# masapasa/qcpinn-convection-diffusion-qiskit

Measured on AMD Instinct MI355X. Metric: collocation-points/sec (PDE+BC+IC loss step), 4-qubit cascade, higher is better.
Workload: dtype f32

## Files before the change

### qcpinn-convection-diffusion-qiskit_amd/csrc/qc_mlp.hip

```cpp
#include "qc_internal.h"
#include "qc_philox.h"

namespace {

__device__ __forceinline__ float qc_tanh(float x) {
  const float e = __expf(2.f * x);
  return 1.f - 2.f * __builtin_amdgcn_rcpf(e + 1.f);
}

typedef float mf2 __attribute__((ext_vector_type(2)));
__device__ __forceinline__ mf2 m_dup(const float a) { return (mf2){a, a}; }
__device__ __forceinline__ mf2 m_fma(const mf2 a, const mf2 b, const mf2 c) { return __builtin_elementwise_fma(a, b, c); }

__device__ __forceinline__ float analytic_u(float t, float x, float y) {
  const float dx = x - 0.5f, dy = y - 0.5f;
  return expf(-100.f * (dx * dx + dy * dy)) * expf(-t);
}
__device__ __forceinline__ float analytic_r(float t, float x, float y, float D, float vx, float vy) {
  const float u = analytic_u(t, x, y);
  const float dx = x - 0.5f, dy = y - 0.5f;
  const float ut = -u, ux = -200.f * dx * u, uy = -200.f * dy * u;
  const float uxx = (40000.f * dx * dx - 400.f) * u;
  const float uyy = (40000.f * dy * dy - 400.f) * u;
  return ut + vx * ux + vy * uy - D * (uxx + uyy);
}

__device__ __forceinline__ float analytic_u_diffusion(float t, float x, float y, float D) {
  const float pi = 3.14159265358979323846f;
  return sinf(pi * x) * sinf(pi * y) * expf(-2.f * pi * pi * D * t);
}

__device__ __forceinline__ float residual_target(const QcPde& pde, float t, float x, float y) {
  return pde.problem != QC_PB_CONVECTION_DIFFUSION ? 0.f : analytic_r(t, x, y, pde.D, pde.vx, pde.vy);
}
__device__ __forceinline__ float value_target(const QcPde& pde, bool seg_a, float t, float x, float y) {
  return pde.problem == QC_PB_PURE_DIFFUSION ? (seg_a ? analytic_u_diffusion(t, x, y, pde.D) : 0.f) : analytic_u(t, x, y);
}

constexpr float QC_PI_F = 3.14159265358979323846f;

template <int NCH>
__device__ __forceinline__ void angle_map_fwd(const float (&v)[NCH], float (&a)[NCH]) {
  const float tau = qc_tanh(v[0]);
  const float ps = QC_PI_F * (1.f - tau * tau);
  a[0] = QC_PI_F * tau;
  if constexpr (NCH == 6) {
    a[1] = ps * v[1];
    a[2] = ps * v[2];
    a[3] = ps * v[3];
    a[4] = ps * (v[4] - 2.f * tau * v[2] * v[2]);
    a[5] = ps * (v[5] - 2.f * tau * v[3] * v[3]);
  }
}

template <int NCH>
__device__ __forceinline__ void angle_map_bwd(const float (&ab)[NCH], const float (&a)[NCH], float (&vb)[NCH]) {
  const float tau = a[0] * (1.f / QC_PI_F);
  const float ps = QC_PI_F * (1.f - tau * tau);
  vb[0] = ps * ab[0];
  if constexpr (NCH == 6) {
    const float tt = 2.f * tau;
    vb[1] = ps * ab[1];
    vb[2] = ps * ab[2] - 2.f * tt * a[2] * ab[4];
    vb[3] = ps * ab[3] - 2.f * tt * a[3] * ab[5];
    vb[4] = ps * ab[4];
    vb[5] = ps * ab[5];
    vb[0] -= tt * (a[1] * ab[1] + a[2] * ab[2] + a[3] * ab[3]) +
             (tt * a[4] + 2.f * a[2] * a[2] * (1.f / QC_PI_F)) * ab[4] +
             (tt * a[5] + 2.f * a[3] * a[3] * (1.f / QC_PI_F)) * ab[5];
  }
}

constexpr int QC_MS = 4;

template <int N, int NCH, int MAP = 0, bool RF = false>
__device__ __forceinline__ void k_pre_fwd_body(const int64_t bid, const float* __restrict__ X, const float* __restrict__ prm,
                                                 QcLayout L, float* __restrict__ ajets, int64_t B,
                                                 const QcDraw* __restrict__ draw = nullptr, float* __restrict__ Xout = nullptr) {
  __shared__ float s_part[QC_MS][NCH * N][64];
  const int lane = threadIdx.x & 63;
  const int wave = __builtin_amdgcn_readfirstlane(threadIdx.x >> 6);
  const int64_t p = (int64_t)bid * 64 + lane;
  const int64_t pc = p < B ? p : B - 1;
  float t, x, y;
  if (draw != nullptr && draw->enabled) {
    if (NCH == 6) qc_draw_point(0, draw->off_res + pc, 0, draw->seed, draw->step, t, x, y);
    else if (pc < draw->n_ic) qc_draw_point(1, draw->off_ic + pc, 0, draw->seed, draw->step, t, x, y);
    else qc_draw_point<RF>(2, draw->off_bc + (pc - draw->n_ic), draw->face_pts, draw->seed, draw->step, t, x, y);
    if (wave == 0 && p < B) {
      Xout[p * 3 + 0] = t;
      Xout[p * 3 + 1] = x;
      Xout[p * 3 + 2] = y;
    }
  } else {
    t = X[pc * 3 + 0];
    x = X[pc * 3 + 1];
    y = X[pc * 3 + 2];
  }
  constexpr int NP2 = NCH == 6 ? 3 : 1;
  mf2 acc2[NP2][N];
#pragma unroll
  for (int cp = 0; cp < NP2; ++cp)
#pragma unroll
    for (int i = 0; i < N; ++i) acc2[cp][i] = (mf2){0.f, 0.f};
  const float* W1 = prm + L.oW1;
  const float* b1 = prm + L.ob1;
  const float* W2 = prm + L.oW2;
  const int hq = (L.H + QC_MS - 1) / QC_MS;
  const int m0 = wave * hq, m1 = (m0 + hq) < L.H ? (m0 + hq) : L.H;
  for (int m = m0; m < m1; ++m) {
    const float w0 = W1[3 * m], w1 = W1[3 * m + 1], w2 = W1[3 * m + 2];
    const float h = fmaf(w0, t, fmaf(w1, x, fmaf(w2, y, b1[m])));
    const float z = qc_tanh(h);
    if constexpr (NCH == 6) {
      const float d1 = 1.f - z * z, d2 = -2.f * z * d1;
      const mf2 zc2[3] = {(mf2){z, d1 * w0}, (mf2){d1 * w1, d1 * w2}, (mf2){d2 * w1 * w1, d2 * w2 * w2}};
#pragma unroll
      for (int i = 0; i < N; ++i) {
        const mf2 wi = m_dup(W2[i * L.H + m]);
#pragma unroll
        for (int cp = 0; cp < 3; ++cp) acc2[cp][i] = m_fma(wi, zc2[cp], acc2[cp][i]);
      }
    } else {
#pragma unroll
      for (int i = 0; i < N; ++i) acc2[0][i].x = fmaf(W2[i * L.H + m], z, acc2[0][i].x);
    }
  }
#pragma unroll
  for (int c = 0; c < NCH; ++c)
#pragma unroll
    for (int i = 0; i < N; ++i) s_part[wave][c * N + i][lane] = (c & 1) ? acc2[c >> 1][i].y : acc2[c >> 1][i].x;
  __syncthreads();
  if (p < B) {
    if constexpr (MAP == 0) {
      for (int f = wave; f < NCH * N; f += QC_MS) {
        float v = (s_part[0][f][lane] + s_part[1][f][lane]) + (s_part[2][f][lane] + s_part[3][f][lane]);
        if (f < N) v += prm[L.ob2 + f];
        ajets[(int64_t)f * B + p] = v;
      }
    } else {
      for (int i = wave; i < N; i += QC_MS) {
        float v[NCH], a[NCH];
#pragma unroll
        for (int c = 0; c < NCH; ++c) {
          const int f = c * N + i;
          v[c] = (s_part[0][f][lane] + s_part[1][f][lane]) + (s_part[2][f][lane] + s_part[3][f][lane]);
        }
        v[0] += prm[L.ob2 + i];
        angle_map_fwd<NCH>(v, a);
#pragma unroll
        for (int c = 0; c < NCH; ++c) ajets[(int64_t)(c * N + i) * B + p] = a[c];
      }
    }
  }
}

template <int N, int NCH, int MAP>
__global__ void __launch_bounds__(256) k_pre_fwd(const float* __restrict__ X, const float* __restrict__ prm,
                                                 QcLayout L, float* __restrict__ ajets, int64_t B) {
  k_pre_fwd_body<N, NCH, MAP>(blockIdx.x, X, prm, L, ajets, B);
}

template <int N, int NCH, int MAP = 0>
__device__ __forceinline__ void k_pre_bwd_body(const int64_t bid, const float* __restrict__ X, const float* __restrict__ prm, QcLayout L,
                          const float* __restrict__ abar, float* __restrict__ part, int64_t part_stride,
                          int64_t row0, int64_t B, int HB, int PS, const float* __restrict__ aj = nullptr) {
  constexpr int NP2 = NCH == 6 ? 3 : 1;
  __shared__ float sX[3][64];
  __shared__ mf2 sA2[NP2 * N][64];
  extern __shared__ float s_acc[];
  const int64_t base = (int64_t)bid * 64;
  const int cnt = (int)((B - base) < 64 ? (B - base) : 64);
  for (int i = threadIdx.x; i < 64 * 3; i += blockDim.x) {
    const int pp = i / 3, k = i % 3;
    sX[k][pp] = pp < cnt ? X[(base + pp) * 3 + k] : 0.f;
  }
  if constexpr (MAP == 0) {
    for (int i = threadIdx.x; i < NCH * N * 64; i += blockDim.x) {
      const int f = i >> 6, pp = i & 63;
      const int c = f / N, w = f % N;
      const float v = pp < cnt ? abar[(int64_t)f * B + base + pp] : 0.f;
      if (c & 1) sA2[(c >> 1) * N + w][pp].y = v;
      else sA2[(c >> 1) * N + w][pp].x = v;
    }
  } else {
    for (int i = threadIdx.x; i < N * 64; i += blockDim.x) {
      const int w = i >> 6, pp = i & 63;
      float ab[NCH], a[NCH], vb[NCH];
#pragma unroll
      for (int c = 0; c < NCH; ++c) {
        const int64_t o = (int64_t)(c * N + w) * B + base + pp;
        ab[c] = pp < cnt ? abar[o] : 0.f;
        a[c] = pp < cnt ? aj[o] : 0.f;
      }
      angle_map_bwd<NCH>(ab, a, vb);
#pragma unroll
      for (int c = 0; c < NCH; ++c) {
        if (c & 1) sA2[(c >> 1) * N + w][pp].y = vb[c];
        else sA2[(c >> 1) * N + w][pp].x = vb[c];
      }
    }
  }
  __syncthreads();

  const int grp = threadIdx.x / HB, m = threadIdx.x % HB;
  const int per = (64 + PS - 1) / PS;
  const int p0 = grp * per, p1 = (p0 + per) < cnt ? (p0 + per) : cnt;
  float gW1[3] = {0.f, 0.f, 0.f}, gb1 = 0.f;
  mf2 gW2p[N];
#pragma unroll
  for (int i = 0; i < N; ++i) gW2p[i] = (mf2){0.f, 0.f};
  if (grp < PS && m < L.H) {
    const float w0 = prm[L.oW1 + 3 * m], w1 = prm[L.oW1 + 3 * m + 1], w2 = prm[L.oW1 + 3 * m + 2];
    const float bb = prm[L.ob1 + m];
    float w2c[N];
#pragma unroll
    for (int i = 0; i < N; ++i) w2c[i] = prm[L.oW2 + i * L.H + m];
    for (int pp = p0; pp < p1; ++pp) {
      const float t = sX[0][pp], x = sX[1][pp], y = sX[2][pp];
      const float h = fmaf(w0, t, fmaf(w1, x, fmaf(w2, y, bb)));
      const float z = qc_tanh(h);
      const float d1 = 1.f - z * z;
      if constexpr (NCH == 6) {
        mf2 a2[3][N], zb2[3];
#pragma unroll
        for (int cp = 0; cp < 3; ++cp) {
          zb2[cp] = (mf2){0.f, 0.f};
#pragma unroll
          for (int i = 0; i < N; ++i) {
            a2[cp][i] = sA2[cp * N + i][pp];
            zb2[cp] = m_fma(m_dup(w2c[i]), a2[cp][i], zb2[cp]);
          }
        }
        const float d2 = -2.f * z * d1;
        const float d3 = -2.f * (d1 * d1 + z * d2);
        const mf2 zc2[3] = {(mf2){z, d1 * w0}, (mf2){d1 * w1, d1 * w2}, (mf2){d2 * w1 * w1, d2 * w2 * w2}};
#pragma unroll
        for (int i = 0; i < N; ++i)
#pragma unroll
          for (int cp = 0; cp < 3; ++cp) gW2p[i] = m_fma(a2[cp][i], zc2[cp], gW2p[i]);
        const float zb[6] = {zb2[0].x, zb2[0].y, zb2[1].x, zb2[1].y, zb2[2].x, zb2[2].y};
        const float hb = zb[0] * d1 + (zb[1] * w0 + zb[2] * w1 + zb[3] * w2) * d2 +
                         (zb[4] * w1 * w1 + zb[5] * w2 * w2) * d3;
        gW1[0] += hb * t + zb[1] * d1;
        gW1[1] += hb * x + zb[2] * d1 + 2.f * zb[4] * d2 * w1;
        gW1[2] += hb * y + zb[3] * d1 + 2.f * zb[5] * d2 * w2;
        gb1 += hb;
      } else {
        float zb0 = 0.f;
#pragma unroll
        for (int i = 0; i < N; ++i) {
          const float a = sA2[i][pp].x;
          zb0 = fmaf(w2c[i], a, zb0);
          gW2p[i].x = fmaf(a, z, gW2p[i].x);
        }
        const float hb = zb0 * d1;
        gW1[0] += hb * t;
        gW1[1] += hb * x;
        gW1[2] += hb * y;
        gb1 += hb;
      }
    }
  }
  if (grp < PS) {
    float* mine = s_acc + (size_t)grp * (4 + N) * HB;
    mine[0 * HB + m] = gW1[0];
    mine[1 * HB + m] = gW1[1];
    mine[2 * HB + m] = gW1[2];
    mine[3 * HB + m] = gb1;
#pragma unroll
    for (int i = 0; i < N; ++i) mine[(4 + i) * HB + m] = gW2p[i].x + gW2p[i].y;
  }
  __syncthreads();
  float* row = part + (row0 + bid) * part_stride;
  if (grp == 0 && m < L.H) {
    float tot[4 + N];
#pragma unroll
    for (int k = 0; k < 4 + N; ++k) {
      float sum = 0.f;
      for (int g2 = 0; g2 < PS; ++g2) sum += s_acc[((size_t)g2 * (4 + N) + k) * HB + m];
      tot[k] = sum;
    }
    row[L.oW1 + 3 * m] = tot[0];
    row[L.oW1 + 3 * m + 1] = tot[1];
    row[L.oW1 + 3 * m + 2] = tot[2];
    row[L.ob1 + m] = tot[3];
#pragma unroll
    for (int i = 0; i < N; ++i) row[L.oW2 + i * L.H + m] = tot[4 + i];
  }
  if (threadIdx.x < N) {
    float sum = 0.f;
// ... 229 lines not shown
    __syncthreads();
    if (live) {
      for (int f = wave; f < NCH * N; f += QC_MS)
        qbar[(int64_t)f * B + p] = (s_buf[0][f][lane] + s_buf[1][f][lane]) + (s_buf[2][f][lane] + s_buf[3][f][lane]);
    }
  }
}

template <int N, int NCH, int MODE>
__global__ void __launch_bounds__(256) k_post(const float* __restrict__ X, const float* __restrict__ prm, QcLayout L,
                                              QcPde pde, const float* __restrict__ qjets,
                                              float* __restrict__ out_u, float* __restrict__ out_res,
                                              const float* __restrict__ in_ubar, const float* __restrict__ in_rbar,
                                              float* __restrict__ qbar, float* __restrict__ part,
                                              int64_t part_stride, int64_t row0, int64_t B) {
  k_post_body<N, NCH, MODE>(blockIdx.x, X, prm, L, pde, qjets, out_u, out_res, in_ubar, in_rbar, qbar, part, part_stride, row0, B);
}

template <int N, int NCH>
__device__ __forceinline__ void k_post_wg_body(const int64_t bid, const float* __restrict__ prm, QcLayout L, QcPde pde, const float* __restrict__ qjets,
                          const float* __restrict__ ubar, const float* __restrict__ rbar,
                          float* __restrict__ part, int64_t part_stride, int64_t row0, int64_t B, int HB, int PS,
                          int gen = 0) {
  __shared__ float sQ[NCH * N][64];
  __shared__ float sU[NCH == 6 ? 6 : 2][64];
  extern __shared__ float s_acc[];
  const int64_t base = (int64_t)bid * 64;
  const int cnt = (int)((B - base) < 64 ? (B - base) : 64);
  for (int i = threadIdx.x; i < NCH * N * 64; i += blockDim.x) {
    const int f = i >> 6, pp = i & 63;
    sQ[f][pp] = pp < cnt ? qjets[(int64_t)f * B + base + pp] : 0.f;
  }
  if (NCH == 6 && gen) {
    for (int i = threadIdx.x; i < 6 * 64; i += blockDim.x) {
      const int k = i >> 6, pp = i & 63;
      sU[k][pp] = pp < cnt ? ubar[(int64_t)k * B + base + pp] : 0.f;
    }
  } else {
    for (int i = threadIdx.x; i < 128; i += blockDim.x) {
      const int k = i >> 6, pp = i & 63;
      const float* src = k == 0 ? ubar : rbar;
      sU[k][pp] = (pp < cnt && src != nullptr) ? src[base + pp] : 0.f;
    }
  }
  __syncthreads();
  const int grp = threadIdx.x / HB, m = threadIdx.x % HB;
  const int per = (64 + PS - 1) / PS;
  const int p0 = grp * per, p1 = (p0 + per) < cnt ? (p0 + per) : cnt;
  float gW3[N], gb3 = 0.f, gW4 = 0.f;
#pragma unroll
  for (int i = 0; i < N; ++i) gW3[i] = 0.f;
  if (grp < PS && m < L.H) {
    float w3[N];
#pragma unroll
    for (int i = 0; i < N; ++i) w3[i] = prm[L.oW3 + m * N + i];
    const float b3m = prm[L.ob3 + m], w4 = prm[L.oW4 + m];
    for (int pp = p0; pp < p1; ++pp) {
      float g[NCH];
#pragma unroll
      for (int c = 0; c < NCH; ++c) {
        float sum = (c == 0) ? b3m : 0.f;
#pragma unroll
        for (int i = 0; i < N; ++i) sum = fmaf(w3[i], sQ[c * N + i][pp], sum);
        g[c] = sum;
      }
      const float z = qc_tanh(g[0]);
      float ub[NCH];
      if (NCH == 6 && gen) {
#pragma unroll
        for (int c = 0; c < NCH; ++c) ub[c] = sU[c < (NCH == 6 ? 6 : 2) ? c : 0][pp];
      } else {
        expand_ub<NCH>(ub, sU[0][pp], sU[1][pp], pde);
      }
      float gb[NCH], gw4;
      post_cotangents<N, NCH>(gb, gw4, g, ub, z, w4);
      gW4 += gw4;
      gb3 += gb[0];
#pragma unroll
      for (int i = 0; i < N; ++i) {
        float sum = gW3[i];
#pragma unroll
        for (int c = 0; c < NCH; ++c) sum = fmaf(gb[c], sQ[c * N + i][pp], sum);
        gW3[i] = sum;
      }
    }
  }
  if (grp < PS) {
    float* mine = s_acc + (size_t)grp * (N + 2) * HB;
#pragma unroll
    for (int i = 0; i < N; ++i) mine[i * HB + m] = gW3[i];
    mine[N * HB + m] = gb3;
    mine[(N + 1) * HB + m] = gW4;
  }
  __syncthreads();
  float* row = part + (row0 + bid) * part_stride;
  if (grp == 0 && m < L.H) {
    float tot[N + 2];
#pragma unroll
    for (int k = 0; k < N + 2; ++k) {
      float sum = 0.f;
      for (int g2 = 0; g2 < PS; ++g2) sum += s_acc[((size_t)g2 * (N + 2) + k) * HB + m];
      tot[k] = sum;
    }
#pragma unroll
    for (int i = 0; i < N; ++i) row[L.oW3 + m * N + i] = tot[i];
    row[L.ob3 + m] = tot[N];
    row[L.oW4 + m] = tot[N + 1];
  }
  if (threadIdx.x == 0) {
    float sum = 0.f;
    for (int pp = 0; pp < cnt; ++pp) sum += sU[0][pp];
    row[L.ob4] = sum;
  }
}

template <int N, int NCH>
__global__ void k_post_wg(const float* __restrict__ prm, QcLayout L, QcPde pde, const float* __restrict__ qjets,
                          const float* __restrict__ ubar, const float* __restrict__ rbar,
                          float* __restrict__ part, int64_t part_stride, int64_t row0, int64_t B, int HB, int PS, int gen) {
  k_post_wg_body<N, NCH>(blockIdx.x, prm, L, pde, qjets, ubar, rbar, part, part_stride, row0, B, HB, PS, gen);
}

template <int N, int MAP = 0, bool RF = false>
__device__ __forceinline__ void k_pre_fwd_value4(const int64_t bid, const float* __restrict__ X, const float* __restrict__ prm,
                                                 QcLayout L, float* __restrict__ ajets, int64_t B,
                                                 const QcDraw* __restrict__ draw, float* __restrict__ Xout) {
  const int lane = threadIdx.x & 63;
  const int wave = __builtin_amdgcn_readfirstlane(threadIdx.x >> 6);
  const int64_t tile = bid * 4 + wave;
  if (tile * 64 >= B) return;
  const int64_t p = tile * 64 + lane;
  const int64_t pc = p < B ? p : B - 1;
  float t, x, y;
  if (draw != nullptr && draw->enabled) {
    if (pc < draw->n_ic) qc_draw_point(1, draw->off_ic + pc, 0, draw->seed, draw->step, t, x, y);
    else qc_draw_point<RF>(2, draw->off_bc + (pc - draw->n_ic), draw->face_pts, draw->seed, draw->step, t, x, y);
    if (p < B) {
      Xout[p * 3 + 0] = t;
      Xout[p * 3 + 1] = x;
      Xout[p * 3 + 2] = y;
    }
  } else {
    t = X[pc * 3 + 0];
    x = X[pc * 3 + 1];
    y = X[pc * 3 + 2];
  }
  const float* W1 = prm + L.oW1;
  const float* b1 = prm + L.ob1;
  const float* W2 = prm + L.oW2;
  const int hq = (L.H + QC_MS - 1) / QC_MS;
  float part[QC_MS][N];
#pragma unroll
  for (int k = 0; k < QC_MS; ++k) {
#pragma unroll
    for (int i = 0; i < N; ++i) part[k][i] = 0.f;
    const int m0 = k * hq, m1 = (m0 + hq) < L.H ? (m0 + hq) : L.H;
    for (int m = m0; m < m1; ++m) {
      const float h = fmaf(W1[3 * m], t, fmaf(W1[3 * m + 1], x, fmaf(W1[3 * m + 2], y, b1[m])));
      const float z = qc_tanh(h);
#pragma unroll
      for (int i = 0; i < N; ++i) part[k][i] = fmaf(W2[i * L.H + m], z, part[k][i]);
    }
  }
  if (p < B) {
#pragma unroll
    for (int i = 0; i < N; ++i) {
      const float v = ((part[0][i] + part[1][i]) + (part[2][i] + part[3][i])) + prm[L.ob2 + i];
      if constexpr (MAP == 0) {
        ajets[(int64_t)i * B + p] = v;
      } else {
        const float vv[1] = {v};
        float a[1];
        angle_map_fwd<1>(vv, a);
        ajets[(int64_t)i * B + p] = a[0];
      }
    }
  }
}

template <int N>
__device__ __forceinline__ void k_post_value4(const int64_t bid, const float* __restrict__ X, const float* __restrict__ prm,
                                              QcLayout L, QcPde pde, const float* __restrict__ qjets,
                                              float* __restrict__ out_u, float* __restrict__ qbar, float* __restrict__ part,
                                              int64_t part_stride, int64_t row0, int64_t B) {
  const int lane = threadIdx.x & 63;
  const int wave = __builtin_amdgcn_readfirstlane(threadIdx.x >> 6);
  const int64_t tile = bid * 4 + wave;
  if (tile * 64 >= B) return;
  const int64_t p = tile * 64 + lane;
  const bool live = p < B;
  const int64_t pc = live ? p : B - 1;
  float q[N];
#pragma unroll
  for (int i = 0; i < N; ++i) q[i] = qjets[(int64_t)i * B + pc];
  const float* W3 = prm + L.oW3;
  const float* b3 = prm + L.ob3;
  const float* W4 = prm + L.oW4;
  const int hq = (L.H + QC_MS - 1) / QC_MS;
  float up[QC_MS], qbu[QC_MS][N];
#pragma unroll
  for (int k = 0; k < QC_MS; ++k) {
    up[k] = 0.f;
#pragma unroll
    for (int i = 0; i < N; ++i) qbu[k][i] = 0.f;
    const int m0 = k * hq, m1 = (m0 + hq) < L.H ? (m0 + hq) : L.H;
    for (int m = m0; m < m1; ++m) {
      float g = b3[m];
#pragma unroll
      for (int i = 0; i < N; ++i) g = fmaf(W3[m * N + i], q[i], g);
      const float z = qc_tanh(g);
      const float w4 = W4[m];
      up[k] = fmaf(w4, z, up[k]);
      const float gb = (1.f - z * z) * w4;
#pragma unroll
      for (int i = 0; i < N; ++i) qbu[k][i] = fmaf(W3[m * N + i], gb, qbu[k][i]);
    }
  }
  const float u = ((up[0] + up[1]) + (up[2] + up[3])) + prm[L.ob4];
  const float t = X[pc * 3 + 0], x = X[pc * 3 + 1], y = X[pc * 3 + 2];
  const bool seg_a = p < pde.n_seg_a;
  const float target = value_target(pde, seg_a, t, x, y);
  const float e = live ? u - target : 0.f;
  const float ub0 = (seg_a ? pde.w_val_a : pde.w_val_b) * e;
  const float la = qc_wave_sum_to_lane63(seg_a ? e * e * pde.inv_n_a : 0.f);
  const float lb = qc_wave_sum_to_lane63(seg_a ? 0.f : e * e * pde.inv_n_b);
  if (lane == 63) {
    float* row = part + (row0 + tile) * part_stride;
    row[L.NP + 0] = 0.f;
    row[L.NP + 1] = lb;
    row[L.NP + 2] = la;
  }
  if (live) {
    out_u[p] = ub0;
#pragma unroll
    for (int i = 0; i < N; ++i)
      qbar[(int64_t)i * B + p] = (ub0 * qbu[0][i] + ub0 * qbu[1][i]) + (ub0 * qbu[2][i] + ub0 * qbu[3][i]);
  }
}

constexpr int QC_POST_VALUE_TPB = 1;

template <int N, int TPB>
__device__ __forceinline__ void k_post_fused_value_body(const int64_t bid, const float* __restrict__ X,
                                                        const float* __restrict__ prm, QcLayout L, QcPde pde,
                                                        const float* __restrict__ qjets, float* __restrict__ out_u,
                                                        float* __restrict__ qbar, float* __restrict__ part,
                                                        int64_t part_stride, int64_t row0, int64_t B,
                                                        float* __restrict__ s_v) {
  constexpr int WPT = QC_MS / TPB, QPW = QC_MS / WPT;
  const int lane = threadIdx.x & 63;
  const int wave = __builtin_amdgcn_readfirstlane(threadIdx.x >> 6);
  const int slot = wave / WPT, wt = wave % WPT;
  const int64_t tile = bid * TPB + slot;
  const bool tile_ok = tile * 64 < B;
  const int64_t p = tile * 64 + lane;
  const bool live = p < B;
  const int64_t pc = live ? p : B - 1;
  float* s_g = s_v + (size_t)slot * (L.H + WPT) * 64;
  float* s_u = s_g + L.H * 64;
  float q[N];
#pragma unroll
  for (int i = 0; i < N; ++i) q[i] = qjets[(int64_t)i * B + pc];
  const float* W3 = prm + L.oW3;
  const float* b3 = prm + L.ob3;
  const float* W4 = prm + L.oW4;
  const int hq = (L.H + QC_MS - 1) / QC_MS;
  const int m0 = tile_ok ? wt * QPW * hq : 0;
  const int m1 = !tile_ok ? 0 : ((m0 + QPW * hq) < L.H ? (m0 + QPW * hq) : L.H);
  float up[QPW];
#pragma unroll
  for (int k = 0; k < QPW; ++k) {
    up[k] = 0.f;
    const int k0 = m0 + k * hq, k1 = (k0 + hq) < m1 ? (k0 + hq) : m1;
    for (int m = k0; m < k1; ++m) {
      float g = b3[m];
#pragma unroll
      for (int i = 0; i < N; ++i) g = fmaf(W3[m * N + i], q[i], g);
      const float z = qc_tanh(g);
      s_g[m * 64 + lane] = z;
      up[k] = fmaf(W4[m], z, up[k]);
    }
  }
  float u;
  if constexpr (QPW == 4) u = (up[0] + up[1]) + (up[2] + up[3]);
  else s_u[wt * 64 + lane] = QPW == 2 ? up[0] + up[1] : up[0];
  __syncthreads();
  if constexpr (WPT == 2) u = s_u[lane] + s_u[64 + lane];
  if constexpr (WPT == 4) u = (s_u[lane] + s_u[64 + lane]) + (s_u[128 + lane] + s_u[192 + lane]);
  u += prm[L.ob4];
  const float t = X[pc * 3 + 0], x = X[pc * 3 + 1], y = X[pc * 3 + 2];
  float* row = part + (row0 + tile) * part_stride;
  const bool seg_a = p < pde.n_seg_a;
  const float target = value_target(pde, seg_a, t, x, y);
  const float e = live ? u - target : 0.f;
  const float ub0 = (seg_a ? pde.w_val_a : pde.w_val_b) * e;
  if (wt == 0 && tile_ok) {
    const float la = qc_wave_sum_to_lane63(seg_a ? e * e * pde.inv_n_a : 0.f);
    const float lb = qc_wave_sum_to_lane63(seg_a ? 0.f : e * e * pde.inv_n_b);
    const float sb4 = qc_wave_sum_to_lane63(ub0);
    if (lane == 63) {
      row[L.NP + 0] = 0.f;
      row[L.NP + 1] = lb;
      row[L.NP + 2] = la;
      row[L.ob4] = sb4;
    }
    if (live) out_u[p] = ub0;
  }
  float ub[1];
  expand_ub<1>(ub, ub0, 0.f, pde);
  for (int m = m0; m < m1; ++m) {
    const float g[1] = {0.f};
    float gb[1], gw4;
    post_cotangents<N, 1>(gb, gw4, g, ub, s_g[m * 64 + lane], W4[m]);
    s_g[m * 64 + lane] = gb[0];
    float wg[N + 2];
#pragma unroll
    for (int i = 0; i < N; ++i) wg[i] = fmaf(gb[0], q[i], 0.f);
    wg[N] = gb[0];
    wg[N + 1] = gw4;
    qc_wave_sum_multi_to_lane63<N + 2>(wg);
    if (lane == 63) {
#pragma unroll
      for (int i = 0; i < N; ++i) row[L.oW3 + m * N + i] = wg[i];
      row[L.ob3 + m] = wg[N];
      row[L.oW4 + m] = wg[N + 1];
    }
  }
  __syncthreads();
  if (live) {
    const int mh = tile_ok ? L.H : 0;
    for (int i = wt; i < N; i += WPT) {
      float qb = 0.f;
      for (int m = 0; m < mh; ++m) qb = fmaf(W3[m * N + i], s_g[m * 64 + lane], qb);
      qbar[(int64_t)i * B + p] = qb;
    }
  }
}


template <int N>
__device__ __forceinline__ void k_post_fused6_body(const int64_t bid, const float* __restrict__ X, const float* __restrict__ prm,
                                                    QcLayout L, QcPde pde, const float* __restrict__ qjets,
                                                    float* __restrict__ out_u, float* __restrict__ out_res,
                                                    float* __restrict__ qbar, float* __restrict__ part, int64_t part_stride,
                                                    int64_t row0, int64_t B, float* __restrict__ s_dyn) {
  constexpr int NCH = 6;
  float* s_z = s_dyn;
  float (*s_u)[NCH][64] = reinterpret_cast<float (*)[NCH][64]>(s_dyn + L.H * 64);
  float (*s_q)[NCH * N][64] = reinterpret_cast<float (*)[NCH * N][64]>(s_dyn);
  const int lane = threadIdx.x & 63;
  const int wave = __builtin_amdgcn_readfirstlane(threadIdx.x >> 6);
  const int64_t tile = bid;
  const int64_t p = tile * 64 + lane;
  const bool live = p < B;
  const int64_t pc = live ? p : B - 1;
  mf2 q2[3][N];
#pragma unroll
  for (int cp = 0; cp < 3; ++cp)
#pragma unroll
    for (int i = 0; i < N; ++i)
      q2[cp][i] = (mf2){qjets[((int64_t)(2 * cp) * N + i) * B + pc], qjets[((int64_t)(2 * cp + 1) * N + i) * B + pc]};
  const float* W3 = prm + L.oW3;
  const float* b3 = prm + L.ob3;
  const float* W4 = prm + L.oW4;
  const int hq = (L.H + QC_MS - 1) / QC_MS;
  const int m0 = wave * hq, m1 = (m0 + hq) < L.H ? (m0 + hq) : L.H;
  auto preact = [&](int m, mf2 (&g2)[3]) {
    g2[0] = (mf2){b3[m], 0.f};
    g2[1] = g2[2] = (mf2){0.f, 0.f};
#pragma unroll
    for (int i = 0; i < N; ++i) {
      const mf2 w = m_dup(W3[m * N + i]);
#pragma unroll
      for (int cp = 0; cp < 3; ++cp) g2[cp] = m_fma(w, q2[cp][i], g2[cp]);
    }
  };
  float u[NCH];
#pragma unroll
  for (int c = 0; c < NCH; ++c) u[c] = 0.f;
  for (int m = m0; m < m1; ++m) {
    mf2 g2[3];
    preact(m, g2);
    const float z = qc_tanh(g2[0].x);
    s_z[m * 64 + lane] = z;
    const float w4 = W4[m];
    const float d1 = 1.f - z * z, d2 = -2.f * z * d1;
    u[0] = fmaf(w4, z, u[0]);
    u[1] = fmaf(w4, d1 * g2[0].y, u[1]);
    u[2] = fmaf(w4, d1 * g2[1].x, u[2]);
    u[3] = fmaf(w4, d1 * g2[1].y, u[3]);
    u[4] = fmaf(w4, d2 * g2[1].x * g2[1].x + d1 * g2[2].x, u[4]);
    u[5] = fmaf(w4, d2 * g2[1].y * g2[1].y + d1 * g2[2].y, u[5]);
  }
#pragma unroll
  for (int c = 0; c < NCH; ++c) s_u[wave][c][lane] = u[c];
  __syncthreads();
#pragma unroll
  for (int c = 0; c < NCH; ++c)
    u[c] = (s_u[0][c][lane] + s_u[1][c][lane]) + (s_u[2][c][lane] + s_u[3][c][lane]);
  u[0] += prm[L.ob4];
  const float t = X[pc * 3 + 0], x = X[pc * 3 + 1], y = X[pc * 3 + 2];
  float* row = part + (row0 + tile) * part_stride;
  const float res = pde.c_t * u[1] + pde.c_x * u[2] + pde.c_y * u[3] - (pde.d_xx * u[4] + pde.d_yy * u[5]);
  const float target = residual_target(pde, t, x, y);
  const float e = live ? res - target : 0.f;
  const float gsc = pde.w_res * e;
  if (wave == 0) {
    const float ls = qc_wave_sum_to_lane63(e * e * pde.inv_n_res);
    if (lane == 63) {
      row[L.NP + 0] = ls;
      row[L.NP + 1] = 0.f;
      row[L.NP + 2] = 0.f;
      row[L.ob4] = 0.f;
    }
    if (live) {
      out_u[p] = 0.f;
      out_res[p] = gsc;
    }
  }
  float ub[NCH];
  expand_ub<NCH>(ub, 0.f, gsc, pde);
  mf2 qb2[3][N];
#pragma unroll
  for (int cp = 0; cp < 3; ++cp)
#pragma unroll
    for (int i = 0; i < N; ++i) qb2[cp][i] = (mf2){0.f, 0.f};
  for (int m = m0; m < m1; ++m) {
    mf2 g2[3];
    preact(m, g2);
    const float g[NCH] = {0.f, g2[0].y, g2[1].x, g2[1].y, g2[2].x, g2[2].y};
    const float z = s_z[m * 64 + lane];
    float gb[NCH], gw4;
    post_cotangents<N, NCH>(gb, gw4, g, ub, z, W4[m]);
    const mf2 gb2[3] = {(mf2){gb[0], gb[1]}, (mf2){gb[2], gb[3]}, (mf2){gb[4], gb[5]}};
    float wg[N + 2];
#pragma unroll
    for (int i = 0; i < N; ++i) {
      const mf2 w3 = m_dup(W3[m * N + i]);
      mf2 acc = gb2[0] * q2[0][i];
#pragma unroll
      for (int cp = 0; cp < 3; ++cp) {
        qb2[cp][i] = m_fma(w3, gb2[cp], qb2[cp][i]);
        if (cp > 0) acc = m_fma(gb2[cp], q2[cp][i], acc);
      }
      wg[i] = acc.x + acc.y;
    }
    wg[N] = gb[0];
    wg[N + 1] = gw4;
    qc_wave_sum_multi_to_lane63<N + 2>(wg);
    if (lane == 63) {
#pragma unroll
      for (int i = 0; i < N; ++i) row[L.oW3 + m * N + i] = wg[i];
      row[L.ob3 + m] = wg[N];
      row[L.oW4 + m] = wg[N + 1];
    }
  }
  __syncthreads();
#pragma unroll
  for (int cp = 0; cp < 3; ++cp)
#pragma unroll
    for (int i = 0; i < N; ++i) {
      s_q[wave][(2 * cp) * N + i][lane] = qb2[cp][i].x;
      s_q[wave][(2 * cp + 1) * N + i][lane] = qb2[cp][i].y;
    }
  __syncthreads();
  if (live) {
    for (int f = wave; f < NCH * N; f += QC_MS)
      qbar[(int64_t)f * B + p] = (s_q[0][f][lane] + s_q[1][f][lane]) + (s_q[2][f][lane] + s_q[3][f][lane]);
  }
}

constexpr int QC_POST_FUSED_MAXH = 128;

static inline size_t qc_post_fused_lds_res(const QcLayout& L) {
  const int a = L.H * 64 + QC_MS * 6 * 64, b = QC_MS * 6 * L.n * 64;
  return (size_t)(a > b ? a : b) * sizeof(float);
}
static inline size_t qc_post_fused_lds_val(const QcLayout& L) {
  return (size_t)QC_POST_VALUE_TPB * (L.H + QC_MS / QC_POST_VALUE_TPB) * 64 * sizeof(float);
}

template <int N, int NCH>
__global__ void __launch_bounds__(256) k_post_fused(const float* __restrict__ X, const float* __restrict__ prm, QcLayout L,
                                                    QcPde pde, const float* __restrict__ qjets, float* __restrict__ out_u,
                                                    float* __restrict__ out_res, float* __restrict__ qbar,
                                                    float* __restrict__ part, int64_t part_stride, int64_t row0, int64_t B) {
  extern __shared__ float s_dyn[];
  if constexpr (NCH == 6) k_post_fused6_body<N>(blockIdx.x, X, prm, L, pde, qjets, out_u, out_res, qbar, part, part_stride, row0, B, s_dyn);
  else k_post_fused_value_body<N, QC_POST_VALUE_TPB>(blockIdx.x, X, prm, L, pde, qjets, out_u, qbar, part, part_stride, row0, B, s_dyn);
}

constexpr int QC_KMAX = 4;

template <int N, int MODE>
__global__ void __launch_bounds__(256) k_post_multi(const float* __restrict__ prm, QcLayout L, int K,
                                                    const float* __restrict__ w4k, const float* __restrict__ qjets,
                                                    float* __restrict__ out_u, const float* __restrict__ ubar,
                                                    float* __restrict__ qbar, float* __restrict__ part, int64_t part_stride,
                                                    float* __restrict__ partk, int64_t partk_stride, int64_t row0, int64_t B) {
  constexpr int NCH = 6;
  __shared__ float s_buf[QC_MS][NCH * (N > QC_KMAX ? N : QC_KMAX)][64];
  const int lane = threadIdx.x & 63;
  const int wave = __builtin_amdgcn_readfirstlane(threadIdx.x >> 6);
  const int64_t tile = blockIdx.x;
  const int64_t p = tile * 64 + lane;
  const bool live = p < B;
  const int64_t pc = live ? p : B - 1;
  float q[NCH][N];
#pragma unroll
  for (int c = 0; c < NCH; ++c)
#pragma unroll
    for (int i = 0; i < N; ++i) q[c][i] = qjets[((int64_t)c * N + i) * B + pc];
  const float* W3 = prm + L.oW3;
  const float* b3 = prm + L.ob3;
  const int H1 = L.H + 1;
  const int hq = (L.H + QC_MS - 1) / QC_MS;
  const int m0 = wave * hq, m1 = (m0 + hq) < L.H ? (m0 + hq) : L.H;
  auto hidden = [&](int m, float (&g)[NCH], float& z, float (&f)[NCH]) {
#pragma unroll
    for (int c = 0; c < NCH; ++c) {
      float sum = (c == 0) ? b3[m] : 0.f;
#pragma unroll
      for (int i = 0; i < N; ++i) sum = fmaf(W3[m * N + i], q[c][i], sum);
      g[c] = sum;
    }
    z = qc_tanh(g[0]);
    const float d1 = 1.f - z * z, d2 = -2.f * z * d1;
    f[0] = z;
    f[1] = d1 * g[1];
    f[2] = d1 * g[2];
    f[3] = d1 * g[3];
    f[4] = d2 * g[2] * g[2] + d1 * g[4];
    f[5] = d2 * g[3] * g[3] + d1 * g[5];
  };
  if constexpr (MODE == 4) {
    float u[QC_KMAX][NCH];
#pragma unroll
    for (int k = 0; k < QC_KMAX; ++k)
#pragma unroll
      for (int c = 0; c < NCH; ++c) u[k][c] = 0.f;
    for (int m = m0; m < m1; ++m) {
      float g[NCH], z, f[NCH];
      hidden(m, g, z, f);
#pragma unroll
      for (int k = 0; k < QC_KMAX; ++k)
        if (k < K) {
          const float w4 = w4k[k * H1 + m];
#pragma unroll
          for (int c = 0; c < NCH; ++c) u[k][c] = fmaf(w4, f[c], u[k][c]);
        }
    }
#pragma unroll
    for (int k = 0; k < QC_KMAX; ++k)
#pragma unroll
      for (int c = 0; c < NCH; ++c) s_buf[wave][k * NCH + c][lane] = u[k][c];
    __syncthreads();
    if (live) {
      for (int f = wave; f < K * NCH; f += QC_MS) {
        float v = (s_buf[0][f][lane] + s_buf[1][f][lane]) + (s_buf[2][f][lane] + s_buf[3][f][lane]);
        if (f % NCH == 0) v += w4k[(f / NCH) * H1 + L.H];
        out_u[(int64_t)f * B + p] = v;
      }
    }
  } else {
    float ub[QC_KMAX][NCH];
#pragma unroll
    for (int k = 0; k < QC_KMAX; ++k)
#pragma unroll
      for (int c = 0; c < NCH; ++c) ub[k][c] = (live && k < K) ? ubar[((int64_t)k * NCH + c) * B + pc] : 0.f;
    float* row = part + (row0 + tile) * part_stride;
    float* rowk = partk + (row0 + tile) * partk_stride;
    if (wave == 0) {
#pragma unroll
      for (int k = 0; k < QC_KMAX; ++k)
        if (k < K) {
          const float sb = qc_wave_sum_to_lane63(ub[k][0]);
          if (lane == 63) rowk[k * H1 + L.H] = sb;
        }
    }
    float qb[NCH][N];
#pragma unroll
    for (int c = 0; c < NCH; ++c)
#pragma unroll
      for (int i = 0; i < N; ++i) qb[c][i] = 0.f;
    for (int m = m0; m < m1; ++m) {
      float g[NCH], z, f[NCH];
      hidden(m, g, z, f);
      float ubw[NCH], gk[QC_KMAX];
#pragma unroll
      for (int c = 0; c < NCH; ++c) ubw[c] = 0.f;
#pragma unroll
      for (int k = 0; k < QC_KMAX; ++k) {
        gk[k] = 0.f;
        if (k < K) {
          const float w4 = w4k[k * H1 + m];
#pragma unroll
          for (int c = 0; c < NCH; ++c) {
            ubw[c] = fmaf(w4, ub[k][c], ubw[c]);
            gk[k] = fmaf(ub[k][c], f[c], gk[k]);
          }
        }
      }
      float gb[NCH], gw4;
      post_cotangents<N, NCH>(gb, gw4, g, ubw, z, 1.f);
      float wg[N + 1];
#pragma unroll
      for (int i = 0; i < N; ++i) {
        const float w3 = W3[m * N + i];
        float sum = 0.f;
#pragma unroll
        for (int c = 0; c < NCH; ++c) {
          qb[c][i] = fmaf(w3, gb[c], qb[c][i]);
          sum = fmaf(gb[c], q[c][i], sum);
        }
        wg[i] = sum;
      }
      wg[N] = gb[0];
      qc_wave_sum_multi_to_lane63<N + 1>(wg);
#pragma unroll
      for (int k = 0; k < QC_KMAX; ++k)
        if (k < K) gk[k] = qc_wave_sum_to_lane63(gk[k]);
// ... 278 lines not shown
```

Baseline: 572.9 million.

## Block and software-prefetch hidden-unit weight loops in MLP pre/post kernels

Adds a generic unit-blocking helper that processes hidden units in blocks of 1, 2 or 4 with optional register prefetch of the next block's weights. It is applied to the pre-forward, post value and post fused6 loops, so that loads overlap with tanh and FMA work and several wave reductions are batched into one multi-value reduction. The LDS partial-sum epilogues are also unrolled so all reads are issued before the global stores. The cost is higher register pressure, which may lower occupancy, and larger code.

```diff
diff --git a/qcpinn-convection-diffusion-qiskit_amd/csrc/qc_mlp.hip b/qcpinn-convection-diffusion-qiskit_amd/csrc/qc_mlp.hip
--- a/qcpinn-convection-diffusion-qiskit_amd/csrc/qc_mlp.hip
+++ b/qcpinn-convection-diffusion-qiskit_amd/csrc/qc_mlp.hip
@@ -72,6 +72,117 @@
 }
 
 constexpr int QC_MS = 4;
+
+template <class Fam, int UB, bool PF, class Load, class Apply>
+__device__ __forceinline__ void qc_unit_blocks(const int m0, const int m1, Load&& load, Apply&& apply) {
+  static_assert(UB == 1 || UB == 2 || UB == 4, "remainder blocks: 2, then 1");
+  int m = m0;
+  const int nblk = m1 > m0 ? (m1 - m0) / UB : 0;
+  if constexpr (PF) {
+    if (nblk > 0) {
+      typename Fam::template Blk<UB> cur;
+      load(cur, m);
+      for (int b = 1; b <= nblk; ++b) {
+        typename Fam::template Blk<UB> nxt;
+        load(nxt, b < nblk ? m + UB : m);
+        apply(cur, m);
+        cur = nxt;
+        m += UB;
+      }
+    }
+  } else {
+    for (int b = 0; b < nblk; ++b, m += UB) {
+      typename Fam::template Blk<UB> w;
+      load(w, m);
+      apply(w, m);
+    }
+  }
+  if constexpr (UB > 2) {
+    if (m + 2 <= m1) {
+      typename Fam::template Blk<2> w;
+      load(w, m);
+      apply(w, m);
+      m += 2;
+    }
+  }
+  if constexpr (UB > 1) {
+    if (m < m1) {
+      typename Fam::template Blk<1> w;
+      load(w, m);
+      apply(w, m);
+    }
+  }
+}
+
+constexpr int qc_pre_ub(int n) { return n <= 4 ? 4 : (n <= 8 ? 2 : 1); }
+
+template <int N>
+struct QcPreW {
+  template <int K>
+  struct Blk { static constexpr int count = K; float w1[3 * K], b1[K], w2[N][K]; };
+};
+
+template <int N, int K>
+__device__ __forceinline__ void pre_blk_load(typename QcPreW<N>::template Blk<K>& w, const float* __restrict__ W1,
+                                             const float* __restrict__ b1, const float* __restrict__ W2, const int H,
+                                             const int m) {
+  const float* __restrict__ p1 = W1 + 3 * m;
+  const float* __restrict__ pb = b1 + m;
+#pragma unroll
+  for (int j = 0; j < 3 * K; ++j) w.w1[j] = p1[j];
+#pragma unroll
+  for (int j = 0; j < K; ++j) w.b1[j] = pb[j];
+#pragma unroll
+  for (int i = 0; i < N; ++i) {
+    const float* __restrict__ p2 = W2 + (i * H + m);
+#pragma unroll
+    for (int j = 0; j < K; ++j) w.w2[i][j] = p2[j];
+  }
+}
+
+template <int N, int NCH, int K>
+__device__ __forceinline__ void pre_blk_apply(const typename QcPreW<N>::template Blk<K>& w, const float t, const float x,
+                                              const float y, mf2 (&acc2)[NCH == 6 ? 3 : 1][N]) {
+  float z[K];
+#pragma unroll
+  for (int j = 0; j < K; ++j)
+    z[j] = qc_tanh(fmaf(w.w1[3 * j], t, fmaf(w.w1[3 * j + 1], x, fmaf(w.w1[3 * j + 2], y, w.b1[j]))));
+#pragma unroll
+  for (int j = 0; j < K; ++j) {
+    if constexpr (NCH == 6) {
+      const float w0 = w.w1[3 * j], w1 = w.w1[3 * j + 1], w2 = w.w1[3 * j + 2];
+      const float d1 = 1.f - z[j] * z[j], d2 = -2.f * z[j] * d1;
+      const mf2 zc2[3] = {(mf2){z[j], d1 * w0}, (mf2){d1 * w1, d1 * w2}, (mf2){d2 * w1 * w1, d2 * w2 * w2}};
+#pragma unroll
+      for (int i = 0; i < N; ++i) {
+        const mf2 wi = m_dup(w.w2[i][j]);
+#pragma unroll
+        for (int cp = 0; cp < 3; ++cp) acc2[cp][i] = m_fma(wi, zc2[cp], acc2[cp][i]);
+      }
+    } else {
+#pragma unroll
+      for (int i = 0; i < N; ++i) acc2[0][i].x = fmaf(w.w2[i][j], z[j], acc2[0][i].x);
+    }
+  }
+}
+
+template <int N, int NCH>
+__device__ __forceinline__ void pre_fwd_units(const float* __restrict__ W1, const float* __restrict__ b1,
+                                              const float* __restrict__ W2, const int H, const int m0, const int m1,
+                                              const float t, const float x, const float y,
+                                              mf2 (&acc2)[NCH == 6 ? 3 : 1][N]) {
+  constexpr int UB = qc_pre_ub(N);
+  qc_unit_blocks<QcPreW<N>, UB, (UB > 1)>(
+      m0, m1,
+      [&](auto& w, const int m) {
+        constexpr int K = std::remove_reference_t<decltype(w)>::count;
+        pre_blk_load<N, K>(w, W1, b1, W2, H, m);
+      },
+      [&](const auto& w, const int) {
+        constexpr int K = std::remove_reference_t<decltype(w)>::count;
+        pre_blk_apply<N, NCH, K>(w, t, x, y, acc2);
+      });
+}
 
 template <int N, int NCH, int MAP = 0, bool RF = false>
 __device__ __forceinline__ void k_pre_fwd_body(const int64_t bid, const float* __restrict__ X, const float* __restrict__ prm,
@@ -108,24 +219,7 @@
   const float* W2 = prm + L.oW2;
   const int hq = (L.H + QC_MS - 1) / QC_MS;
   const int m0 = wave * hq, m1 = (m0 + hq) < L.H ? (m0 + hq) : L.H;
-  for (int m = m0; m < m1; ++m) {
-    const float w0 = W1[3 * m], w1 = W1[3 * m + 1], w2 = W1[3 * m + 2];
-    const float h = fmaf(w0, t, fmaf(w1, x, fmaf(w2, y, b1[m])));
-    const float z = qc_tanh(h);
-    if constexpr (NCH == 6) {
-      const float d1 = 1.f - z * z, d2 = -2.f * z * d1;
-      const mf2 zc2[3] = {(mf2){z, d1 * w0}, (mf2){d1 * w1, d1 * w2}, (mf2){d2 * w1 * w1, d2 * w2 * w2}};
-#pragma unroll
-      for (int i = 0; i < N; ++i) {
-        const mf2 wi = m_dup(W2[i * L.H + m]);
-#pragma unroll
-        for (int cp = 0; cp < 3; ++cp) acc2[cp][i] = m_fma(wi, zc2[cp], acc2[cp][i]);
-      }
-    } else {
-#pragma unroll
-      for (int i = 0; i < N; ++i) acc2[0][i].x = fmaf(W2[i * L.H + m], z, acc2[0][i].x);
-    }
-  }
+  pre_fwd_units<N, NCH>(W1, b1, W2, L.H, m0, m1, t, x, y, acc2);
 #pragma unroll
   for (int c = 0; c < NCH; ++c)
 #pragma unroll
@@ -133,10 +227,28 @@
   __syncthreads();
   if (p < B) {
     if constexpr (MAP == 0) {
-      for (int f = wave; f < NCH * N; f += QC_MS) {
-        float v = (s_part[0][f][lane] + s_part[1][f][lane]) + (s_part[2][f][lane] + s_part[3][f][lane]);
-        if (f < N) v += prm[L.ob2 + f];
-        ajets[(int64_t)f * B + p] = v;
+      constexpr int NF = (NCH * N + QC_MS - 1) / QC_MS;
+      if constexpr (NF <= 12) {
+        float v[NF];
+#pragma unroll
+        for (int j = 0; j < NF; ++j) {
+          const int f = wave + QC_MS * j, fc = f < NCH * N ? f : 0;
+          v[j] = (s_part[0][fc][lane] + s_part[1][fc][lane]) + (s_part[2][fc][lane] + s_part[3][fc][lane]);
+        }
+#pragma unroll
+        for (int j = 0; j < NF; ++j) {
+          const int f = wave + QC_MS * j;
+          if (f < NCH * N) {
+            if (f < N) v[j] += prm[L.ob2 + f];
+            ajets[(int64_t)f * B + p] = v[j];
+          }
+        }
+      } else {
+        for (int f = wave; f < NCH * N; f += QC_MS) {
+          float v = (s_part[0][f][lane] + s_part[1][f][lane]) + (s_part[2][f][lane] + s_part[3][f][lane]);
+          if (f < N) v += prm[L.ob2 + f];
+          ajets[(int64_t)f * B + p] = v;
+        }
       }
     } else {
       for (int i = wave; i < N; i += QC_MS) {
@@ -672,15 +784,13 @@
   float part[QC_MS][N];
 #pragma unroll
   for (int k = 0; k < QC_MS; ++k) {
-#pragma unroll
-    for (int i = 0; i < N; ++i) part[k][i] = 0.f;
+    mf2 acc[1][N];
+#pragma unroll
+    for (int i = 0; i < N; ++i) acc[0][i] = (mf2){0.f, 0.f};
     const int m0 = k * hq, m1 = (m0 + hq) < L.H ? (m0 + hq) : L.H;
-    for (int m = m0; m < m1; ++m) {
-      const float h = fmaf(W1[3 * m], t, fmaf(W1[3 * m + 1], x, fmaf(W1[3 * m + 2], y, b1[m])));
-      const float z = qc_tanh(h);
-#pragma unroll
-      for (int i = 0; i < N; ++i) part[k][i] = fmaf(W2[i * L.H + m], z, part[k][i]);
-    }
+    pre_fwd_units<N, 1>(W1, b1, W2, L.H, m0, m1, t, x, y, acc);
+#pragma unroll
+    for (int i = 0; i < N; ++i) part[k][i] = acc[0][i].x;
   }
   if (p < B) {
 #pragma unroll
@@ -759,6 +869,34 @@
 }
 
 constexpr int QC_POST_VALUE_TPB = 1;
+
+template <int N>
+struct QcPostW {
+  template <int K>
+  struct Blk { static constexpr int count = K; float w3[K][N], b3[K], w4[K]; };
+};
+template <int N, int K>
+__device__ __forceinline__ void post_blk_load(typename QcPostW<N>::template Blk<K>& w, const float* __restrict__ W3,
+                                              const float* __restrict__ b3, const float* __restrict__ W4, const int m) {
+  const float* __restrict__ p3 = W3 + m * N;
+  const float* __restrict__ pb = b3 + m;
+  const float* __restrict__ p4 = W4 + m;
+#pragma unroll
+  for (int j = 0; j < K; ++j)
+#pragma unroll
+    for (int i = 0; i < N; ++i) w.w3[j][i] = p3[j * N + i];
+#pragma unroll
+  for (int j = 0; j < K; ++j) w.b3[j] = pb[j];
+#pragma unroll
+  for (int j = 0; j < K; ++j) w.w4[j] = p4[j];
+}
+struct QcColW {
+  template <int K>
+  struct Blk { static constexpr int count = K; float c[K]; };
+};
+constexpr int qc_post_ub_a(int n) { return n == 3 ? 2 : (n <= 4 ? 4 : (n <= 8 ? 2 : 1)); }
+constexpr bool qc_post_pf(int n) { return n <= 8; }
+constexpr int qc_post_ub_vb(int n) { return n <= 8 ? 2 : 1; }
 
 template <int N, int TPB>
 __device__ __forceinline__ void k_post_fused_value_body(const int64_t bid, const float* __restrict__ X,
@@ -792,14 +930,25 @@
   for (int k = 0; k < QPW; ++k) {
     up[k] = 0.f;
     const int k0 = m0 + k * hq, k1 = (k0 + hq) < m1 ? (k0 + hq) : m1;
-    for (int m = k0; m < k1; ++m) {
-      float g = b3[m];
-#pragma unroll
-      for (int i = 0; i < N; ++i) g = fmaf(W3[m * N + i], q[i], g);
-      const float z = qc_tanh(g);
-      s_g[m * 64 + lane] = z;
-      up[k] = fmaf(W4[m], z, up[k]);
-    }
+    qc_unit_blocks<QcPostW<N>, qc_post_ub_a(N), qc_post_pf(N)>(
+        k0, k1,
+        [&](auto& w, const int m) { post_blk_load<N, std::remove_reference_t<decltype(w)>::count>(w, W3, b3, W4, m); },
+        [&](const auto& w, const int m) {
+          constexpr int K = std::remove_reference_t<decltype(w)>::count;
+          float z[K];
+#pragma unroll
+          for (int j = 0; j < K; ++j) {
+            float g = w.b3[j];
+#pragma unroll
+            for (int i = 0; i < N; ++i) g = fmaf(w.w3[j][i], q[i], g);
+            z[j] = qc_tanh(g);
+          }
+#pragma unroll
+          for (int j = 0; j < K; ++j) {
+            s_g[(m + j) * 64 + lane] = z[j];
+            up[k] = fmaf(w.w4[j], z[j], up[k]);
+          }
+        });
   }
   float u;
   if constexpr (QPW == 4) u = (up[0] + up[1]) + (up[2] + up[3]);
@@ -828,35 +977,66 @@
   }
   float ub[1];
   expand_ub<1>(ub, ub0, 0.f, pde);
-  for (int m = m0; m < m1; ++m) {
-    const float g[1] = {0.f};
-    float gb[1], gw4;
-    post_cotangents<N, 1>(gb, gw4, g, ub, s_g[m * 64 + lane], W4[m]);
-    s_g[m * 64 + lane] = gb[0];
-    float wg[N + 2];
-#pragma unroll
-    for (int i = 0; i < N; ++i) wg[i] = fmaf(gb[0], q[i], 0.f);
-    wg[N] = gb[0];
-    wg[N + 1] = gw4;
-    qc_wave_sum_multi_to_lane63<N + 2>(wg);
-    if (lane == 63) {
-#pragma unroll
-      for (int i = 0; i < N; ++i) row[L.oW3 + m * N + i] = wg[i];
-      row[L.ob3 + m] = wg[N];
-      row[L.oW4 + m] = wg[N + 1];
-    }
-  }
+  qc_unit_blocks<QcColW, qc_post_ub_vb(N), false>(
+      m0, m1,
+      [&](auto& w, const int m) {
+#pragma unroll
+        for (int j = 0; j < std::remove_reference_t<decltype(w)>::count; ++j) w.c[j] = W4[m + j];
+      },
+      [&](const auto& w, const int m) {
+        constexpr int K = std::remove_reference_t<decltype(w)>::count;
+        float wg[K * (N + 2)];
+#pragma unroll
+        for (int j = 0; j < K; ++j) {
+          const float g[1] = {0.f};
+          float gb[1], gw4;
+          post_cotangents<N, 1>(gb, gw4, g, ub, s_g[(m + j) * 64 + lane], w.c[j]);
+          s_g[(m + j) * 64 + lane] = gb[0];
+#pragma unroll
+          for (int i = 0; i < N; ++i) wg[j * (N + 2) + i] = fmaf(gb[0], q[i], 0.f);
+          wg[j * (N + 2) + N] = gb[0];
+          wg[j * (N + 2) + N + 1] = gw4;
+        }
+        qc_wave_sum_multi_to_lane63<K * (N + 2)>(wg);
+        if (lane == 63) {
+#pragma unroll
+          for (int j = 0; j < K; ++j) {
+#pragma unroll
+            for (int i = 0; i < N; ++i) row[L.oW3 + (m + j) * N + i] = wg[j * (N + 2) + i];
+            row[L.ob3 + m + j] = wg[j * (N + 2) + N];
+            row[L.oW4 + m + j] = wg[j * (N + 2) + N + 1];
+          }
+        }
+      });
   __syncthreads();
   if (live) {
     const int mh = tile_ok ? L.H : 0;
     for (int i = wt; i < N; i += WPT) {
       float qb = 0.f;
-      for (int m = 0; m < mh; ++m) qb = fmaf(W3[m * N + i], s_g[m * 64 + lane], qb);
+      qc_unit_blocks<QcColW, 4, true>(
+          0, mh,
+          [&](auto& w, const int m) {
+#pragma unroll
+            for (int j = 0; j < std::remove_reference_t<decltype(w)>::count; ++j) w.c[j] = W3[(m + j) * N + i];
+          },
+          [&](const auto& w, const int m) {
+            constexpr int K = std::remove_reference_t<decltype(w)>::count;
+            float gbv[K];
+#pragma unroll
+            for (int j = 0; j < K; ++j) gbv[j] = s_g[(m + j) * 64 + lane];
+#pragma unroll
+            for (int j = 0; j < K; ++j) qb = fmaf(w.c[j], gbv[j], qb);
+          });
       qbar[(int64_t)i * B + p] = qb;
     }
   }
 }
 
+
+template <int N> constexpr int QC_POST6_UB_A = qc_post_ub_a(N);
+template <int N> constexpr bool QC_POST6_PF_A = qc_post_pf(N);
+template <int N> constexpr int QC_POST6_UB_B = 1;
+template <int N> constexpr bool QC_POST6_PF_B = false;
 
 template <int N>
 __device__ __forceinline__ void k_post_fused6_body(const int64_t bid, const float* __restrict__ X, const float* __restrict__ prm,
@@ -885,33 +1065,43 @@
   const float* W4 = prm + L.oW4;
   const int hq = (L.H + QC_MS - 1) / QC_MS;
   const int m0 = wave * hq, m1 = (m0 + hq) < L.H ? (m0 + hq) : L.H;
-  auto preact = [&](int m, mf2 (&g2)[3]) {
-    g2[0] = (mf2){b3[m], 0.f};
+  auto preact = [&](const float (&w3)[N], const float b3m, mf2 (&g2)[3]) {
+    g2[0] = (mf2){b3m, 0.f};
     g2[1] = g2[2] = (mf2){0.f, 0.f};
 #pragma unroll
     for (int i = 0; i < N; ++i) {
-      const mf2 w = m_dup(W3[m * N + i]);
+      const mf2 w = m_dup(w3[i]);
 #pragma unroll
       for (int cp = 0; cp < 3; ++cp) g2[cp] = m_fma(w, q2[cp][i], g2[cp]);
     }
+  };
+  auto load_blk = [&](auto& w, const int m) {
+    post_blk_load<N, std::remove_reference_t<decltype(w)>::count>(w, W3, b3, W4, m);
   };
   float u[NCH];
 #pragma unroll
   for (int c = 0; c < NCH; ++c) u[c] = 0.f;
-  for (int m = m0; m < m1; ++m) {
-    mf2 g2[3];
-    preact(m, g2);
-    const float z = qc_tanh(g2[0].x);
-    s_z[m * 64 + lane] = z;
-    const float w4 = W4[m];
-    const float d1 = 1.f - z * z, d2 = -2.f * z * d1;
-    u[0] = fmaf(w4, z, u[0]);
-    u[1] = fmaf(w4, d1 * g2[0].y, u[1]);
-    u[2] = fmaf(w4, d1 * g2[1].x, u[2]);
-    u[3] = fmaf(w4, d1 * g2[1].y, u[3]);
-    u[4] = fmaf(w4, d2 * g2[1].x * g2[1].x + d1 * g2[2].x, u[4]);
-    u[5] = fmaf(w4, d2 * g2[1].y * g2[1].y + d1 * g2[2].y, u[5]);
-  }
+  qc_unit_blocks<QcPostW<N>, QC_POST6_UB_A<N>, QC_POST6_PF_A<N>>(m0, m1, load_blk, [&](const auto& w, const int m) {
+    constexpr int K = std::remove_reference_t<decltype(w)>::count;
+    mf2 g2[K][3];
+    float z[K];
+#pragma unroll
+    for (int j = 0; j < K; ++j) preact(w.w3[j], w.b3[j], g2[j]);
+#pragma unroll
+    for (int j = 0; j < K; ++j) z[j] = qc_tanh(g2[j][0].x);
+#pragma unroll
+    for (int j = 0; j < K; ++j) {
+      s_z[(m + j) * 64 + lane] = z[j];
+      const float w4 = w.w4[j];
+      const float d1 = 1.f - z[j] * z[j], d2 = -2.f * z[j] * d1;
+      u[0] = fmaf(w4, z[j], u[0]);
+      u[1] = fmaf(w4, d1 * g2[j][0].y, u[1]);
+      u[2] = fmaf(w4, d1 * g2[j][1].x, u[2]);
+      u[3] = fmaf(w4, d1 * g2[j][1].y, u[3]);
+      u[4] = fmaf(w4, d2 * g2[j][1].x * g2[j][1].x + d1 * g2[j][2].x, u[4]);
+      u[5] = fmaf(w4, d2 * g2[j][1].y * g2[j][1].y + d1 * g2[j][2].y, u[5]);
+    }
+  });
 #pragma unroll
   for (int c = 0; c < NCH; ++c) s_u[wave][c][lane] = u[c];
   __syncthreads();
@@ -945,36 +1135,43 @@
   for (int cp = 0; cp < 3; ++cp)
 #pragma unroll
     for (int i = 0; i < N; ++i) qb2[cp][i] = (mf2){0.f, 0.f};
-  for (int m = m0; m < m1; ++m) {
-    mf2 g2[3];
-    preact(m, g2);
-    const float g[NCH] = {0.f, g2[0].y, g2[1].x, g2[1].y, g2[2].x, g2[2].y};
-    const float z = s_z[m * 64 + lane];
-    float gb[NCH], gw4;
-    post_cotangents<N, NCH>(gb, gw4, g, ub, z, W4[m]);
-    const mf2 gb2[3] = {(mf2){gb[0], gb[1]}, (mf2){gb[2], gb[3]}, (mf2){gb[4], gb[5]}};
-    float wg[N + 2];
-#pragma unroll
-    for (int i = 0; i < N; ++i) {
-      const mf2 w3 = m_dup(W3[m * N + i]);
-      mf2 acc = gb2[0] * q2[0][i];
-#pragma unroll
-      for (int cp = 0; cp < 3; ++cp) {
-        qb2[cp][i] = m_fma(w3, gb2[cp], qb2[cp][i]);
-        if (cp > 0) acc = m_fma(gb2[cp], q2[cp][i], acc);
-      }
-      wg[i] = acc.x + acc.y;
-    }
-    wg[N] = gb[0];
-    wg[N + 1] = gw4;
-    qc_wave_sum_multi_to_lane63<N + 2>(wg);
+  qc_unit_blocks<QcPostW<N>, QC_POST6_UB_B<N>, QC_POST6_PF_B<N>>(m0, m1, load_blk, [&](const auto& w, const int m) {
+    constexpr int K = std::remove_reference_t<decltype(w)>::count;
+    float wg[K * (N + 2)];
+#pragma unroll
+    for (int j = 0; j < K; ++j) {
+      mf2 g2[3];
+      preact(w.w3[j], w.b3[j], g2);
+      const float g[NCH] = {0.f, g2[0].y, g2[1].x, g2[1].y, g2[2].x, g2[2].y};
+      const float z = s_z[(m + j) * 64 + lane];
+      float gb[NCH], gw4;
+      post_cotangents<N, NCH>(gb, gw4, g, ub, z, w.w4[j]);
+      const mf2 gb2[3] = {(mf2){gb[0], gb[1]}, (mf2){gb[2], gb[3]}, (mf2){gb[4], gb[5]}};
+#pragma unroll
+      for (int i = 0; i < N; ++i) {
+        const mf2 w3 = m_dup(w.w3[j][i]);
+        mf2 acc = gb2[0] * q2[0][i];
+#pragma unroll
+        for (int cp = 0; cp < 3; ++cp) {
+          qb2[cp][i] = m_fma(w3, gb2[cp], qb2[cp][i]);
+          if (cp > 0) acc = m_fma(gb2[cp], q2[cp][i], acc);
+        }
+        wg[j * (N + 2) + i] = acc.x + acc.y;
+      }
+      wg[j * (N + 2) + N] = gb[0];
+      wg[j * (N + 2) + N + 1] = gw4;
+    }
+    qc_wave_sum_multi_to_lane63<K * (N + 2)>(wg);
     if (lane == 63) {
 #pragma unroll
-      for (int i = 0; i < N; ++i) row[L.oW3 + m * N + i] = wg[i];
-      row[L.ob3 + m] = wg[N];
-      row[L.oW4 + m] = wg[N + 1];
-    }
-  }
+      for (int j = 0; j < K; ++j) {
+#pragma unroll
+        for (int i = 0; i < N; ++i) row[L.oW3 + (m + j) * N + i] = wg[j * (N + 2) + i];
+        row[L.ob3 + m + j] = wg[j * (N + 2) + N];
+        row[L.oW4 + m + j] = wg[j * (N + 2) + N + 1];
+      }
+    }
+  });
   __syncthreads();
 #pragma unroll
   for (int cp = 0; cp < 3; ++cp)
@@ -985,8 +1182,23 @@
     }
   __syncthreads();
   if (live) {
-    for (int f = wave; f < NCH * N; f += QC_MS)
-      qbar[(int64_t)f * B + p] = (s_q[0][f][lane] + s_q[1][f][lane]) + (s_q[2][f][lane] + s_q[3][f][lane]);
+    constexpr int NF = (NCH * N + QC_MS - 1) / QC_MS;
+    if constexpr (NF <= 12) {
+      float v[NF];
+#pragma unroll
+      for (int j = 0; j < NF; ++j) {
+        const int f = wave + QC_MS * j, fc = f < NCH * N ? f : 0;
+        v[j] = (s_q[0][fc][lane] + s_q[1][fc][lane]) + (s_q[2][fc][lane] + s_q[3][fc][lane]);
+      }
+#pragma unroll
+      for (int j = 0; j < NF; ++j) {
+        const int f = wave + QC_MS * j;
+        if (f < NCH * N) qbar[(int64_t)f * B + p] = v[j];
+      }
+    } else {
+      for (int f = wave; f < NCH * N; f += QC_MS)
+        qbar[(int64_t)f * B + p] = (s_q[0][f][lane] + s_q[1][f][lane]) + (s_q[2][f][lane] + s_q[3][f][lane]);
+    }
   }
 }
 
```

Result: faster. 586.4 million, median of 6 (+2.4%).
